# aipixel/GPS-Gaussian

Measured on NVIDIA H100. Metric: novel_views_per_sec_1024sq_500kgauss, higher is better.
Workload: dtype f32

## Files before the change

### gps-gaussian_b200/_lib.py

```python
import ctypes as C
import os
import threading

import torch

_HERE = os.path.dirname(os.path.abspath(__file__))
LIB_PATH = os.path.join(_HERE, "lib", "libgpsg_sm90.so")


class GpsgError(RuntimeError):
    pass


class RasterSettings(C.Structure):
    _fields_ = [("image_height", C.c_int32), ("image_width", C.c_int32), ("tanfovx", C.c_float),
                ("tanfovy", C.c_float), ("bg", C.c_float * 3), ("scale_modifier", C.c_float),
                ("viewmatrix", C.c_float * 16), ("projmatrix", C.c_float * 16), ("sh_degree", C.c_int32),
                ("campos", C.c_float * 3), ("prefiltered", C.c_int32), ("debug", C.c_int32)]


class GeomView(C.Structure):
    _fields_ = [("depths", C.c_void_p), ("means2D", C.c_void_p), ("conic_opacity", C.c_void_p),
                ("tiles_touched", C.c_void_p), ("point_offsets", C.c_void_p)]


class BinningView(C.Structure):
    _fields_ = [("point_list_keys", C.c_void_p), ("point_list", C.c_void_p), ("slabA", C.c_void_p), ("block_lists", C.c_void_p)]


class ImageView(C.Structure):
    _fields_ = [("final_T", C.c_void_p), ("n_contrib", C.c_void_p), ("ranges", C.c_void_p), ("block_counts", C.c_void_p)]


ALLOC_FN = C.CFUNCTYPE(C.c_void_p, C.c_void_p, C.c_size_t)

if not os.path.exists(LIB_PATH):
    raise ImportError(
        f"{LIB_PATH} not found: the CUDA extension is not built. Run `python gps-gaussian_b200/build.py` "
        "(nvcc, sm_90a). There is deliberately no CPU / PyTorch fallback.")

lib = C.CDLL(LIB_PATH)

_vp, _i, _i64, _sz = C.c_void_p, C.c_int, C.c_int64, C.c_size_t
lib.gpsg_last_error.restype = C.c_char_p
lib.gpsg_last_error.argtypes = []
lib.gpsg_version.restype = _i
_pp = C.POINTER(C.c_void_p)
_rs = C.POINTER(RasterSettings)
lib.gpsg_rasterize_forward.restype = _i
lib.gpsg_rasterize_forward.argtypes = [_rs, _i, _vp, _i, _i] + [_vp] * 11 + [
    ALLOC_FN, _vp, ALLOC_FN, _vp, ALLOC_FN, _vp, C.POINTER(C.c_int32), _i]
lib.gpsg_rasterize_forward_maps_begin.restype = _i
lib.gpsg_rasterize_forward_maps_begin.argtypes = [_rs, _i, _vp, _i] + [_pp] * 6 + [
    _vp, ALLOC_FN, _vp, ALLOC_FN, _vp, _vp, _i]
lib.gpsg_rasterize_forward_maps_finish.restype = _i
lib.gpsg_rasterize_forward_maps_finish.argtypes = [_rs, _i, _vp, _i] + [_pp] * 6 + [_vp] * 6 + [
    ALLOC_FN, _vp, _vp, C.POINTER(C.c_int32)]
lib.gpsg_rasterize_forward_planned.restype = _i
lib.gpsg_rasterize_forward_planned.argtypes = [_rs, _i, _vp, _i] + [_vp] * 12 + [_i64, _vp, _vp, _i]
lib.gpsg_rasterize_forward_maps_planned.restype = _i
lib.gpsg_rasterize_forward_maps_planned.argtypes = [_rs, _i, _vp, _i] + [_pp] * 6 + [_vp] * 6 + [_i64, _vp, _vp, _i]
lib.gpsg_rasterize_backward_workspace_bytes.restype = _sz
lib.gpsg_rasterize_backward_workspace_bytes.argtypes = [_i, _i64, _i, _i]
lib.gpsg_rasterize_backward.restype = _i
lib.gpsg_rasterize_backward.argtypes = [_rs, _i, _vp, _i, _i, C.c_int32] + [_vp] * 23 + [_i]
lib.gpsg_rasterize_backward_maps_workspace_bytes.restype = _sz
lib.gpsg_rasterize_backward_maps_workspace_bytes.argtypes = [_i, _i64, _i, _i]
lib.gpsg_rasterize_backward_maps.restype = _i
lib.gpsg_rasterize_backward_maps.argtypes = [_rs, _i, _vp, _i, C.c_int32] + [_pp] * 6 + [_vp] * 7 + [_pp] * 5 + [_vp, _i]
lib.gpsg_mark_visible.restype = _i
lib.gpsg_mark_visible.argtypes = [_i, _vp, _i, _vp, C.POINTER(C.c_float), _vp]
lib.gpsg_geom_view.restype = _i
lib.gpsg_geom_view.argtypes = [_vp, _i, C.POINTER(GeomView)]
lib.gpsg_binning_view.restype = _i
lib.gpsg_binning_view.argtypes = [_vp, _i64, C.POINTER(BinningView)]
lib.gpsg_image_view.restype = _i
lib.gpsg_image_view.argtypes = [_vp, _i, _i, C.POINTER(ImageView)]
lib.gpsg_corr_sampler_forward.restype = _i
lib.gpsg_corr_sampler_forward.argtypes = [_i, _vp, _i, _i, _i, _i, _i, _vp, _i64, _i64, _i64, _vp, _i64, _i, _vp]
lib.gpsg_corr_sampler_backward.restype = _i
lib.gpsg_corr_sampler_backward.argtypes = [_i, _vp, _i, _i, _i, _i, _i, _vp, _i64, _vp, _i, _vp]

lib.gpsg_raster_geom_bytes.restype = _sz
lib.gpsg_raster_geom_bytes.argtypes = [_i]
lib.gpsg_raster_binning_bytes.restype = _sz
lib.gpsg_raster_binning_bytes.argtypes = [_i64]
lib.gpsg_raster_image_bytes.restype = _sz
lib.gpsg_raster_image_bytes.argtypes = [_i, _i]
lib.gpsg_corr_build_pyramid.restype = _i
lib.gpsg_corr_build_pyramid.argtypes = [_i, _vp, _i, _i, _i, _i, _i, _i, _vp, _vp, C.POINTER(C.c_void_p), _i]
lib.gpsg_corr_build_backward.restype = _i
lib.gpsg_corr_build_backward.argtypes = [_i, _vp, _i, _i, _i, _i, _i, _i, _vp, _vp, _vp, _vp, _vp]
lib.gpsg_corr_lookup_pyramid_forward.restype = _i
lib.gpsg_corr_lookup_pyramid_forward.argtypes = [_i, _vp, _i, _i, _i, _i, C.POINTER(C.c_void_p), C.POINTER(C.c_int32), _i,
                                                 _vp, _i64, _i, _vp]
lib.gpsg_corr_lookup_pyramid_backward.restype = _i
lib.gpsg_corr_lookup_pyramid_backward.argtypes = [_i, _vp, _i, _i, _i, _i, C.POINTER(C.c_void_p), C.POINTER(C.c_int32), _i,
                                                  _vp, _i64, _i, _vp]
lib.gpsg_unproject_forward.restype = _i
lib.gpsg_unproject_forward.argtypes = [_i, _vp, _i, _i, _vp, _vp, _i64, _vp, _vp, _i, _vp, _vp, _vp, _vp, _vp]
lib.gpsg_unproject_backward.restype = _i
lib.gpsg_unproject_backward.argtypes = [_i, _vp, _i, _i, _vp, _vp, _i64, _vp, _vp, _i, _vp, _vp, _vp, _vp, _vp]
lib.gpsg_l1_ssim_workspace_bytes.restype = _sz
lib.gpsg_l1_ssim_workspace_bytes.argtypes = [_i, _i, _i]
lib.gpsg_l1_ssim_forward.restype = _i
lib.gpsg_l1_ssim_forward.argtypes = [_i, _vp, _i, _i, _i, _vp, _vp, C.c_float, C.c_float, _vp, _vp, _vp]
lib.gpsg_l1_ssim_backward.restype = _i
lib.gpsg_l1_ssim_backward.argtypes = [_i, _vp, _i, _i, _i, _vp, _vp, _vp, C.c_float, C.c_float, _vp, _vp]
lib.gpsg_point_splat_workspace_bytes.restype = _sz
lib.gpsg_point_splat_workspace_bytes.argtypes = [_i, _i]
lib.gpsg_point_splat.restype = _i
lib.gpsg_point_splat.argtypes = [_i, _vp, _i, _i, _i, _i64, _vp, _vp, _vp, _vp, _vp]


class RectifyCamera(C.Structure):
    _fields_ = [("K", C.c_double * 9), ("R", C.c_double * 9), ("P", C.c_double * 9)]


class RectifyPlanes(C.Structure):
    _fields_ = [(n, C.c_void_p) for n in ("img", "mask", "depth", "img_out", "mask_out", "depth_out", "img_tensor",
                                          "mask_tensor")]


MESH_MAX_CAMERAS = 8
MESH_MAX_LIGHTS = 16


class Mesh(C.Structure):
    _fields_ = [("verts", C.c_void_p), ("face_verts", C.c_void_p), ("uvs", C.c_void_p), ("face_uvs", C.c_void_p),
                ("tex", C.c_void_p), ("num_verts", C.c_int32), ("num_faces", C.c_int32), ("num_uvs", C.c_int32),
                ("tex_w", C.c_int32), ("tex_h", C.c_int32)]


class MeshCamera(C.Structure):
    _fields_ = [("width", C.c_int32), ("height", C.c_int32), ("fx", C.c_float), ("fy", C.c_float), ("cx", C.c_float),
                ("cy", C.c_float), ("pos", C.c_float * 3), ("inv_rot", C.c_float * 9), ("img", C.c_void_p),
                ("zbuf", C.c_void_p), ("mask", C.c_void_p)]


class MeshScene(C.Structure):
    _fields_ = [("cameras", MeshCamera * MESH_MAX_CAMERAS), ("light_dir", (C.c_float * 3) * MESH_MAX_LIGHTS),
                ("light_color", (C.c_float * 3) * MESH_MAX_LIGHTS), ("num_cameras", C.c_int32),
                ("num_lights", C.c_int32)]


lib.gpsg_mesh_render_workspace_bytes.restype = _sz
lib.gpsg_mesh_render_workspace_bytes.argtypes = [_i, _i64]
lib.gpsg_mesh_render.restype = _i
lib.gpsg_mesh_render.argtypes = [_i, _vp, Mesh, MeshScene, _vp, _sz]
lib.gpsg_rectify_remap.restype = _i
lib.gpsg_rectify_remap.argtypes = [_i, _vp, C.POINTER(RectifyCamera), _i, _i, _i, _i, _i, _i, C.POINTER(RectifyPlanes)]
lib.gpsg_rectify_flow.restype = _i
lib.gpsg_rectify_flow.argtypes = [_i, _vp, _i, _i, _i, C.c_double, C.c_double, C.c_double, _pp, _pp, _pp, _pp]
class SeqLossArgs(C.Structure):
    _fields_ = [("pred", C.c_void_p * 32), ("grad", C.c_void_p * 32), ("weight", C.c_float * 32), ("gt", C.c_void_p),
                ("valid", C.c_void_p), ("numel", C.c_int64), ("n_pred", C.c_int), ("gt_dtype", C.c_int)]


SEQ_LOSS_MAX_PRED = 32
GS_HEAD_PARAMS = ("out_w", "out_b", "rot_w1", "rot_b1", "rot_w2", "rot_b2", "scale_w1", "scale_b1", "scale_w2",
                  "scale_b2", "opacity_w1", "opacity_b1", "opacity_w2", "opacity_b2")
lib.gpsg_convex_upsample_forward.restype = _i
lib.gpsg_convex_upsample_forward.argtypes = [_i, _vp, _i, _i, _i, _i, _i, _i, _vp, _vp, _vp]
lib.gpsg_convex_upsample_backward_workspace_bytes.restype = _sz
lib.gpsg_convex_upsample_backward_workspace_bytes.argtypes = [_i, _i, _i, _i]
lib.gpsg_convex_upsample_backward.restype = _i
lib.gpsg_convex_upsample_backward.argtypes = [_i, _vp, _i, _i, _i, _i, _i, _i, _vp, _vp, _vp, _vp, _vp, _vp]
lib.gpsg_sequence_loss_workspace_bytes.restype = _sz
lib.gpsg_sequence_loss_workspace_bytes.argtypes = []
lib.gpsg_sequence_loss_forward.restype = _i
lib.gpsg_sequence_loss_forward.argtypes = [_i, _vp, SeqLossArgs, _vp, _vp]
lib.gpsg_sequence_loss_backward.restype = _i
lib.gpsg_sequence_loss_backward.argtypes = [_i, _vp, SeqLossArgs, _vp, _vp]


class GsHeadWeights(C.Structure):
    _fields_ = [(n, C.c_void_p) for n in GS_HEAD_PARAMS]


lib.gpsg_gs_head_workspace_bytes.restype = _sz
lib.gpsg_gs_head_workspace_bytes.argtypes = [_i, _i, _i]
lib.gpsg_gs_head_forward.restype = _i
lib.gpsg_gs_head_forward.argtypes = [_i, _vp, _i, _i, _i] + [_vp] * 6 + [GsHeadWeights, _vp]


class GsHeadGrads(C.Structure):
    _fields_ = [(n, C.c_void_p) for n in GS_HEAD_PARAMS]


lib.gpsg_gs_head_backward_workspace_bytes.restype = _sz
lib.gpsg_gs_head_backward_workspace_bytes.argtypes = [_i, _i, _i]
lib.gpsg_gs_head_backward.restype = _i
lib.gpsg_gs_head_backward.argtypes = [_i, _vp, _i, _i, _i] + [_vp] * 9 + [GsHeadWeights, GsHeadGrads, _vp]
ENCODER_STEM_PARAMS = ("in_conv_w", "in_conv_b", "in_norm_w", "in_norm_b") + tuple(
    f"b{k}_{n}" for k in (1, 2) for n in ("conv1_w", "conv1_b", "norm1_w", "norm1_b", "conv2_w", "conv2_b", "norm2_w",
                                          "norm2_b"))
ENCODER_STEM_TF32, ENCODER_STEM_FP16 = 0, 1


class EncoderStemWeights(C.Structure):
    _fields_ = [(n, C.c_void_p) for n in ENCODER_STEM_PARAMS]


lib.gpsg_encoder_stem_workspace_bytes.restype = _sz
lib.gpsg_encoder_stem_workspace_bytes.argtypes = [_i, _i, _i, _i, _i]
lib.gpsg_encoder_stem_forward.restype = _i
lib.gpsg_encoder_stem_forward.argtypes = [_i, _vp, _i, _i, _i, _i, _i, _vp, EncoderStemWeights, _vp, _vp]
lib.gpsg_profile_enable.restype = _i
lib.gpsg_profile_enable.argtypes = [_i]
lib.gpsg_profile_read.restype = _i
lib.gpsg_profile_read.argtypes = [C.POINTER(C.c_float), C.POINTER(C.c_int32), C.POINTER(C.c_int32), _i]
lib.gpsg_profile_stage_name.restype = C.c_char_p
lib.gpsg_profile_stage_name.argtypes = [_i]

EXPORTED = ["gpsg_last_error", "gpsg_version", "gpsg_rasterize_forward", "gpsg_rasterize_forward_maps_begin",
            "gpsg_rasterize_forward_maps_finish", "gpsg_raster_geom_bytes", "gpsg_raster_binning_bytes",
            "gpsg_raster_image_bytes", "gpsg_rasterize_forward_planned", "gpsg_rasterize_forward_maps_planned",
            "gpsg_rasterize_backward_workspace_bytes", "gpsg_rasterize_backward",
            "gpsg_rasterize_backward_maps_workspace_bytes", "gpsg_rasterize_backward_maps", "gpsg_mark_visible",
            "gpsg_geom_view", "gpsg_binning_view", "gpsg_image_view", "gpsg_corr_sampler_forward",
            "gpsg_corr_sampler_backward", "gpsg_corr_build_pyramid", "gpsg_corr_build_backward",
            "gpsg_corr_lookup_pyramid_forward", "gpsg_corr_lookup_pyramid_backward", "gpsg_unproject_forward",
            "gpsg_unproject_backward", "gpsg_l1_ssim_workspace_bytes", "gpsg_l1_ssim_forward", "gpsg_l1_ssim_backward",
            "gpsg_set_corr_build", "gpsg_profile_enable", "gpsg_profile_read", "gpsg_profile_stage_name",
            "gpsg_point_splat_workspace_bytes", "gpsg_point_splat", "gpsg_rectify_remap", "gpsg_rectify_flow",
            "gpsg_convex_upsample_forward", "gpsg_convex_upsample_backward_workspace_bytes",
            "gpsg_convex_upsample_backward", "gpsg_sequence_loss_workspace_bytes", "gpsg_sequence_loss_forward",
            "gpsg_sequence_loss_backward", "gpsg_mesh_render_workspace_bytes", "gpsg_mesh_render", "gpsg_jpeg_parse",
            "gpsg_jpeg_decode_workspace_bytes", "gpsg_jpeg_decode", "gpsg_jpeg_encode_max_bytes",
            "gpsg_jpeg_encode_workspace_bytes", "gpsg_jpeg_encode", "gpsg_gs_head_workspace_bytes",
            "gpsg_gs_head_forward", "gpsg_gs_head_backward_workspace_bytes", "gpsg_gs_head_backward",
            "gpsg_encoder_stem_workspace_bytes", "gpsg_encoder_stem_forward"]

BWD_DETERMINISTIC = 1
FWD_ANTIALIAS = 1


def forward_flags(antialiasing=False):
    return FWD_ANTIALIAS if antialiasing else 0


def check(rc, what):
    if rc != 0:
        msg = lib.gpsg_last_error()
        raise GpsgError(f"{what} failed (code {rc}): {msg.decode() if msg else ''}")


_tls = threading.local()


def _alloc_trampoline(user, nbytes):
    try:
        t = torch.empty(int(nbytes), dtype=torch.uint8, device=_tls.device)
        _tls.bufs[int(user or 0)] = t
        return t.data_ptr()
    except Exception:
        return None


ALLOC_CB = ALLOC_FN(_alloc_trampoline)


def begin_alloc(device):
    _tls.device = device
    _tls.bufs = {}


def end_alloc():
    bufs = _tls.bufs
    _tls.bufs = {}
    return bufs


def device_stream(device):
    device = torch.device(device)
    idx = device.index if device.index is not None else torch.cuda.current_device()
    return idx, C.c_void_p(torch.cuda.current_stream(idx).cuda_stream)


def _ptr(t):
    return C.c_void_p(t.data_ptr()) if (t is not None and t.numel() > 0) else None


def rasterize_forward(settings, out_color, radii, means3D, opacities, colors_precomp=None, shs=None, scales=None,
                      rotations=None, cov3D_precomp=None, out_depth=None, out_alpha=None, antialiasing=False):
    if (out_depth is None) != (out_alpha is None):
        raise ValueError("out_depth and out_alpha must be given together")
    dev = means3D.device
    idx, stream = device_stream(dev)
    n = C.c_int32(0)
    fn = lib.gpsg_rasterize_forward
    begin_alloc(dev)
    try:
        with torch.cuda.device(dev):
            rc = fn(
                C.byref(settings), idx, stream, int(means3D.shape[0]), int(shs.shape[1]) if shs is not None else 0,
                _ptr(means3D), _ptr(colors_precomp), _ptr(shs), _ptr(opacities), _ptr(scales), _ptr(rotations),
                _ptr(cov3D_precomp), _ptr(out_color), _ptr(out_depth), _ptr(out_alpha), _ptr(radii), ALLOC_CB, C.c_void_p(1),
                ALLOC_CB, C.c_void_p(2), ALLOC_CB, C.c_void_p(3), C.byref(n), forward_flags(antialiasing))
    finally:
        bufs = end_alloc()
    check(rc, fn.__name__)
    return int(n.value), (bufs.get(1), bufs.get(2), bufs.get(3))


def backward_flags(deterministic=None):
    if deterministic is None:
        deterministic = torch.are_deterministic_algorithms_enabled()
    return BWD_DETERMINISTIC if deterministic else 0

# ... 55 lines not shown
```

### gps-gaussian_b200/build.py

```python
import os
import subprocess
import sys
from concurrent.futures import ThreadPoolExecutor

HERE = os.path.dirname(os.path.abspath(__file__))
CSRC = os.path.join(HERE, "csrc")
OBJ = os.path.join(HERE, "build")
LIBDIR = os.path.join(HERE, "lib")
LIB = os.path.join(LIBDIR, "libgpsg_sm90.so")

ARCH = ["-gencode", "arch=compute_90a,code=sm_90a"]
COMMON = ["-O3", "-std=c++17", "-lineinfo", "-Xcompiler", "-fPIC", "-Xcompiler", "-fvisibility=hidden",
          "--expt-relaxed-constexpr", "-Xptxas", "-v"]
SOURCES = {
    "gpsg_capi.cu": [],
    "raster_preprocess.cu": ["-fmad=false"],
    "raster_binning.cu": [],
    "raster_render.cu": [],
    "raster_backward.cu": [],
    "corr.cu": [],
    "corr_tc.cu": [],
    "sh.cu": [],
    "unproject.cu": [],
    "loss.cu": [],
    "point_splat.cu": [],
    "rectify.cu": ["-fmad=false"],
    "flow_head.cu": [],
    "gs_head.cu": [],
    "encoder_stem.cu": [],
    "mesh_render.cu": ["-fmad=false"],
    "jpeg_decode.cu": [],
    "jpeg_encode.cu": [],
}


def _nvcc():
    for cand in (os.environ.get("NVCC"), "/usr/local/cuda/bin/nvcc", "nvcc"):
        if cand and (os.path.isabs(cand) and os.path.exists(cand) or not os.path.isabs(cand)):
            return cand
    return "nvcc"


def _deps(src):
    hdrs = [os.path.join(CSRC, f) for f in os.listdir(CSRC) if f.endswith((".cuh", ".h"))]
    hdrs.append(os.path.join(os.path.dirname(HERE), "include", "gpsg.h"))
    return [src, os.path.abspath(__file__)] + hdrs


def _stale(dst, deps):
    if not os.path.exists(dst):
        return True
    t = os.path.getmtime(dst)
    return any(os.path.getmtime(d) > t for d in deps)


def _compile(name, extra, force, verbose):
    src = os.path.join(CSRC, name)
    obj = os.path.join(OBJ, name.replace(".cu", ".o"))
    if not force and not _stale(obj, _deps(src)):
        return obj, ""
    cmd = [_nvcc()] + ARCH + COMMON + extra + ["-c", src, "-o", obj]
    p = subprocess.run(cmd, capture_output=True, text=True)
    log = " ".join(cmd) + "\n" + p.stdout + p.stderr
    if p.returncode != 0:
        raise RuntimeError(log)
    with open(obj + ".log", "w") as f:
        f.write(log)
    if verbose:
        print(log)
    return obj, log


def build(force=False, verbose=False):
    os.makedirs(OBJ, exist_ok=True)
    os.makedirs(LIBDIR, exist_ok=True)
    with ThreadPoolExecutor(max_workers=len(SOURCES)) as ex:
        res = list(ex.map(lambda kv: _compile(kv[0], kv[1], force, verbose), SOURCES.items()))
    objs = [r[0] for r in res]
    if force or _stale(LIB, objs):
        cmd = [_nvcc()] + ARCH + ["-shared", "-o", LIB] + objs + ["-Xcompiler", "-fvisibility=hidden", "-cudart",
                                                                  "static"]
        p = subprocess.run(cmd, capture_output=True, text=True)
        if p.returncode != 0:
            raise RuntimeError(" ".join(cmd) + "\n" + p.stdout + p.stderr)
    return LIB


if __name__ == "__main__":
    print(build(force="--force" in sys.argv, verbose="--verbose" in sys.argv))
```

### gps-gaussian_b200/csrc/raster_binning.cu

```cuda
#include <cub/cub.cuh>
#include "gpsg_internal.cuh"
#include "tile_scan.cuh"

namespace gpsg {

size_t scan_temp_bytes(int P) {
    size_t bytes = 0;
    cub::DeviceScan::InclusiveSum(nullptr, bytes, (uint32_t*)nullptr, (uint32_t*)nullptr, P > 0 ? P : 1);
    return bytes;
}

size_t sort_temp_bytes(size_t N, int end_bit) {
    size_t bytes = 0;
    cub::DeviceRadixSort::SortPairs(nullptr, bytes, (uint64_t*)nullptr, (uint64_t*)nullptr, (uint32_t*)nullptr,
                                    (uint32_t*)nullptr, (int64_t)(N > 0 ? N : 1), 0, end_bit);
    return bytes;
}

int run_scan(GeomState g, int P, cudaStream_t stream) {
    if (P <= 0) return GPSG_OK;
    size_t bytes = g.scan_temp_bytes;
    GPSG_CUDA(cub::DeviceScan::InclusiveSum(g.scan_temp, bytes, g.tiles_touched, g.point_offsets, P, stream));
    return GPSG_OK;
}

__global__ void __launch_bounds__(256) duplicate_kernel(const __grid_constant__ Camera cam, int P,
                                                        const int32_t* __restrict__ radii, GeomState g,
                                                        BinningState b) {
    const int i = blockIdx.x * blockDim.x + threadIdx.x;
    if (i >= P) return;
    const int radius = radii[i];
    if (radius <= 0) return;
    uint32_t off = (i == 0) ? 0u : g.point_offsets[i - 1];
    int rx0, ry0, rx1, ry1;
    tile_rect(cam.grid_x, cam.grid_y, g.means2D[i], radius, rx0, ry0, rx1, ry1);
    const uint64_t dbits = (uint64_t)__float_as_uint(g.depths[i]);
    for (int y = ry0; y < ry1; ++y)
        for (int x = rx0; x < rx1; ++x) {
            const uint64_t key = ((uint64_t)(uint32_t)(y * cam.grid_x + x) << 32) | dbits;
            b.keys_unsorted[off] = key;
            b.vals_unsorted[off] = (uint32_t)i;
            ++off;
        }
}

int launch_duplicate(const Camera& cam, int P, const int32_t* radii, GeomState g, BinningState b, cudaStream_t stream) {
    if (P <= 0) return GPSG_OK;
    duplicate_kernel<<<(P + 255) / 256, 256, 0, stream>>>(cam, P, radii, g, b);
    GPSG_LAUNCH_CHECK();
    return GPSG_OK;
}

int run_sort(BinningState b, size_t N, int end_bit, cudaStream_t stream) {
    if (N == 0) return GPSG_OK;
    size_t bytes = b.sort_temp_bytes;
    GPSG_CUDA(cub::DeviceRadixSort::SortPairs(b.sort_temp, bytes, b.keys_unsorted, b.keys, b.vals_unsorted, b.vals,
                                              (int64_t)N, 0, end_bit, stream));
    return GPSG_OK;
}



__global__ void __launch_bounds__(256) tile_scan_kernel(int tiles, ImageState im, uint32_t capacity) {
    tile_scan_block(tiles, im, capacity);
}

int launch_tile_scan(const Camera& cam, ImageState im, uint32_t capacity, cudaStream_t stream) {
    tile_scan_kernel<<<1, 256, 0, stream>>>(cam.grid_x * cam.grid_y, im, capacity);
    GPSG_LAUNCH_CHECK();
    return GPSG_OK;
}

__global__ void __launch_bounds__(256) bucket_scatter_kernel(const __grid_constant__ Camera cam, int P,
                                                             const int32_t* __restrict__ radii, GeomState g,
                                                             BinningState b, ImageState im) {
    __shared__ uint32_t sh_cnt[kBoxBins];
    __shared__ uint32_t sh_base[kBoxBins];
    __shared__ int s_bb[4];
    if (im.totals[2]) return;
    if (threadIdx.x == 0) { s_bb[0] = 0x7fffffff; s_bb[1] = 0x7fffffff; s_bb[2] = 0; s_bb[3] = 0; }
    for (int t = threadIdx.x; t < kBoxBins; t += blockDim.x) sh_cnt[t] = 0u;
    __syncthreads();
    const int i = blockIdx.x * blockDim.x + threadIdx.x;
    int rx0 = 0, ry0 = 0, rx1 = 0, ry1 = 0;
    uint2 entry = make_uint2(0u, 0u);
    if (i < P) {
        const int radius = radii[i];
        if (radius > 0) {
            tile_rect(cam.grid_x, cam.grid_y, g.means2D[i], radius, rx0, ry0, rx1, ry1);
            entry = make_uint2((uint32_t)i, __float_as_uint(g.depths[i]));
        }
    }
    TileBox box;
    if (!cta_tile_box(rx0, ry0, rx1, ry1, s_bb, box)) {
        for (int y = ry0; y < ry1; ++y)
            for (int x = rx0; x < rx1; ++x) {
                const int t = y * cam.grid_x + x;
                b.bucket[im.ranges[t].x + atomicAdd(&im.tile_cursor[t], 1u)] = entry;
            }
        return;
    }
    for (int y = ry0; y < ry1; ++y)
        for (int x = rx0; x < rx1; ++x) atomicAdd(&sh_cnt[(y - box.y0) * box.w + (x - box.x0)], 1u);
    __syncthreads();
    for (int t = threadIdx.x; t < box.w * box.h; t += blockDim.x) {
        const uint32_t c = sh_cnt[t];
        if (c) {
            const int tile = (box.y0 + t / box.w) * cam.grid_x + box.x0 + t % box.w;
            sh_base[t] = im.ranges[tile].x + atomicAdd(&im.tile_cursor[tile], c);
            sh_cnt[t] = 0u;
        }
    }
    __syncthreads();
    for (int y = ry0; y < ry1; ++y)
        for (int x = rx0; x < rx1; ++x) {
            const int t = (y - box.y0) * box.w + (x - box.x0);
            b.bucket[sh_base[t] + atomicAdd(&sh_cnt[t], 1u)] = entry;
        }
}

int launch_bucket_scatter(const Camera& cam, int P, const int32_t* radii, GeomState g, BinningState b, ImageState im,
                          cudaStream_t stream) {
    if (P <= 0) return GPSG_OK;
    bucket_scatter_kernel<<<(P + 255) / 256, 256, 0, stream>>>(cam, P, radii, g, b, im);
    GPSG_LAUNCH_CHECK();
    return GPSG_OK;
}

__device__ __forceinline__ void slab_entry(uint32_t id, const GaussianSrc& src, const GeomState& g, float4& A,
                                           float4& B, float4& C) {
    const float2 xy = g.means2D[id];
    const float4 co = g.conic_opacity[id];
    float r, gg, bb;
    src_color(src, id, r, gg, bb);
    float ex = 3.0e38f, ey = 3.0e38f;
    const float detc = co.x * co.z - co.y * co.y;
    if (!(co.w * 255.0f >= 1.0f)) {
        ex = ey = -3.0e38f;
    } else if (detc > 0.0f && co.x > 0.0f && co.z > 0.0f) {
        const float tau2 = 2.0f * __logf(co.w * 255.0f) * 1.0005f + 1e-4f;
        ex = sqrtf(tau2 * co.z / detc) * 1.0005f + 0.01f;
        ey = sqrtf(tau2 * co.x / detc) * 1.0005f + 0.01f;
        if (!(ex == ex) || !(ey == ey)) { ex = 3.0e38f; ey = 3.0e38f; }
    }
    A = make_float4(xy.x, xy.y, ex, ey);
    const float kL = 1.4426950408889634f;
    B = make_float4(-0.5f * kL * co.x, -kL * co.y, -0.5f * kL * co.z, co.w);
    C = make_float4(r, gg, bb, __uint_as_float(id));
}

constexpr int kSortThreads = 512;
constexpr int kSortCTAsPerSM = 3;


__device__ __forceinline__ uint32_t block_hit_mask(const float4& a, int tile_x, int tile_y) {
    bool hx[2], hy[4];
#pragma unroll
    for (int c = 0; c < 2; ++c) {
        const float wx0 = (float)(tile_x * GPSG_TILE_X + 8 * c), wx1 = (float)(tile_x * GPSG_TILE_X + 8 * c + 7);
        hx[c] = (a.x >= wx0 - a.z) && (a.x <= wx1 + a.z);
    }
#pragma unroll
    for (int w = 0; w < 4; ++w) {
        const float wy0 = (float)(tile_y * GPSG_TILE_Y + 4 * w), wy1 = (float)(tile_y * GPSG_TILE_Y + 4 * w + 3);
        hy[w] = (a.y >= wy0 - a.w) && (a.y <= wy1 + a.w);
    }
    uint32_t hits = 0u;
#pragma unroll
    for (int k = 0; k < 8; ++k) hits |= (uint32_t)(hx[fwd_block_col(k)] && hy[fwd_block_row(k)]) << k;
    return hits;
}

__device__ __forceinline__ void append_block_list(const uint8_t* hits, uint32_t r0, uint32_t m, int k,
                                                  uint32_t* __restrict__ list, uint32_t& base) {
    const int lane = threadIdx.x & 31;
    const unsigned lt = (1u << lane) - 1u;
#pragma unroll 4
    for (uint32_t c = 0; c < m; c += 32) {
        const uint32_t i = c + lane;
        const bool hit = i < m && ((hits[i] >> k) & 1u);
        const unsigned mask = __ballot_sync(0xffffffffu, hit);
        if (hit) list[base + __popc(mask & lt)] = r0 + i;
        base += __popc(mask);
    }
}

constexpr int kBigItems = (int)kMaxTileSort / kSortThreads;
template <int ITEMS>
struct TileSort {
    using BRS = cub::BlockRadixSort<uint32_t, kSortThreads, ITEMS, uint32_t, 4, false>;
    union Smem {
        typename BRS::TempStorage sort;
        unsigned long long keys[kSortThreads * ITEMS];
    };

    static constexpr int kMaxRun = 16;
    __device__ static void run(Smem& sm, uint32_t* flags, uint8_t* hits, const uint2* __restrict__ src, int n, int id_bits,
                               uint32_t tile, int grid_x, size_t out0, const GaussianSrc& src_in, const GeomState& g,
                               const BinningState& b, uint32_t* __restrict__ blk_count) {
        uint32_t keys[ITEMS], ids[ITEMS];
        uint32_t dmin = ~0u, dmax = 0u;
#pragma unroll
        for (int k = 0; k < ITEMS; ++k) {
            const int i = k * kSortThreads + (int)threadIdx.x;
            const uint2 e = i < n ? src[i] : make_uint2(0u, 0u);
            ids[k] = e.x;
            keys[k] = e.y;
            if (i < n) { dmin = min(dmin, e.y); dmax = max(dmax, e.y); }
        }
        dmin = __reduce_min_sync(0xffffffffu, dmin);
        dmax = __reduce_max_sync(0xffffffffu, dmax);
        if (threadIdx.x == 0) { flags[0] = ~0u; flags[1] = 0u; flags[2] = 0u; }
        __syncthreads();
        if ((threadIdx.x & 31) == 0) { atomicMin(&flags[0], dmin); atomicMax(&flags[1], dmax); }
        __syncthreads();
        const uint32_t dlo = flags[0];
        const int w = 32 - __clz(flags[1] - dlo);
        const uint32_t pad = 1u << w;
#pragma unroll
        for (int k = 0; k < ITEMS; ++k) keys[k] = (k * kSortThreads + (int)threadIdx.x) < n ? keys[k] - dlo : pad;
        BRS(sm.sort).SortBlockedToStriped(keys, ids, 0, w + 1);
        __syncthreads();
#pragma unroll
        for (int k = 0; k < ITEMS; ++k)
            sm.keys[k * kSortThreads + (int)threadIdx.x] = ((unsigned long long)(keys[k] + dlo) << 32) | ids[k];
        __syncthreads();
        bool redo = false;
#pragma unroll 1
        for (int k = 0; k < ITEMS; ++k) {
            const int r = k * kSortThreads + (int)threadIdx.x;
            if (r + 1 < n) {
                const uint32_t d = (uint32_t)(sm.keys[r] >> 32);
                const bool start = (r == 0 || (uint32_t)(sm.keys[r - 1] >> 32) != d) && (uint32_t)(sm.keys[r + 1] >> 32) == d;
                if (start) {
                    int e = r + 1;
                    while (e + 1 < n && (uint32_t)(sm.keys[e + 1] >> 32) == d) ++e;
                    if (e - r + 1 > kMaxRun) redo = true;
                    else
                        for (int a = r + 1; a <= e; ++a) {
                            const unsigned long long v = sm.keys[a];
                            int c = a - 1;
                            while (c >= r && sm.keys[c] > v) { sm.keys[c + 1] = sm.keys[c]; --c; }
                            sm.keys[c + 1] = v;
                        }
                }
            }
        }
        if (redo) flags[2] = 1u;
        __syncthreads();
        if (flags[2]) {
#pragma unroll
            for (int k = 0; k < ITEMS; ++k) {
                const int r = k * kSortThreads + (int)threadIdx.x;
                const unsigned long long v = sm.keys[r];
                ids[k] = (uint32_t)v;
                keys[k] = r < n ? (uint32_t)(v >> 32) - dlo : pad;
            }
            __syncthreads();
            BRS(sm.sort).SortBlockedToStriped(ids, keys, 0, id_bits);
            __syncthreads();
#pragma unroll
            for (int k = 0; k < ITEMS; ++k)
                sm.keys[k * kSortThreads + (int)threadIdx.x] = ((unsigned long long)keys[k] << 32) | ids[k];
            __syncthreads();
#pragma unroll
            for (int k = 0; k < ITEMS; ++k) {
                const unsigned long long v = sm.keys[(int)threadIdx.x * ITEMS + k];
                ids[k] = (uint32_t)v;
                keys[k] = (uint32_t)(v >> 32);
            }
            __syncthreads();
            BRS(sm.sort).SortBlockedToStriped(keys, ids, 0, w + 1);
            __syncthreads();
#pragma unroll
            for (int k = 0; k < ITEMS; ++k)
                sm.keys[k * kSortThreads + (int)threadIdx.x] = ((unsigned long long)(keys[k] + dlo) << 32) | ids[k];
            __syncthreads();
        }
        const unsigned long long tile_hi = (unsigned long long)tile << 32;
        const int tile_y = (int)tile / grid_x, tile_x = (int)tile - tile_y * grid_x;
#pragma unroll 1
        for (int k = 0; k < ITEMS; ++k) {
            const int r = k * kSortThreads + (int)threadIdx.x;
            if (r < n) {
                const unsigned long long v = sm.keys[r];
                const uint32_t id = (uint32_t)v;
                const size_t o = out0 + r;
                if (b.keys) {
                    b.keys[o] = tile_hi | (v >> 32);
                    b.vals[o] = id;
                }
                float4 A, B, C;
                slab_entry(id, src_in, g, A, B, C);
                b.slabA[o] = A;
                b.slabB[o] = B;
                b.slabC[o] = C;
                hits[r] = (uint8_t)block_hit_mask(A, tile_x, tile_y);
            }
        }
        __syncthreads();
        const int warp = (int)threadIdx.x >> 5, blk = warp & 7;
        const uint32_t split = ((uint32_t)n / 2u) & ~127u;
        uint32_t* __restrict__ list = b.blk_list + 8 * out0 + (size_t)blk * n;
        uint32_t cnt = 0u;
        if (warp < 8) {
            append_block_list(hits, 0u, split, blk, list, cnt);
        } else {
            const uint32_t* __restrict__ words = reinterpret_cast<const uint32_t*>(hits);
#pragma unroll 1
            for (uint32_t i = threadIdx.x & 31; i < split / 4u; i += 32) cnt += __popc(words[i] & (0x01010101u << blk));
            cnt = __reduce_add_sync(0xffffffffu, cnt);
            append_block_list(hits + split, split, (uint32_t)n - split, blk, list, cnt);
            if ((threadIdx.x & 31) == 0) blk_count[8 * (size_t)tile + blk] = cnt;
        }
    }
};

template <bool BIG>
__global__ void __launch_bounds__(kSortThreads, BIG ? 1 : kSortCTAsPerSM) tile_sort_gather_kernel(const GaussianSrc colors, GeomState g,
                                                                            BinningState b, ImageState im, int id_bits,
                                                                            int grid_x, uint32_t tiles) {
    __shared__ uint32_t flags[4];
    if (im.totals[2]) return;
    if constexpr (BIG) {
        __shared__ typename TileSort<kBigItems>::Smem t16;
        __shared__ __align__(16) uint8_t hits[kSortThreads * kBigItems];
        const uint32_t nbig = im.totals[3];
        for (uint32_t k = blockIdx.x; k < nbig; k += gridDim.x) {
            const uint32_t tile = im.big_tiles[k];
            const uint2 range = im.ranges[tile];
            const int n = (int)(range.y - range.x);
            TileSort<kBigItems>::run(t16, flags, hits, b.bucket + range.x, n, id_bits, tile, grid_x, range.x, colors, g, b,
                                     im.blk_count);
            __syncthreads();
        }
    } else {
        __shared__ union {
            typename TileSort<1>::Smem t1;
            typename TileSort<2>::Smem t2;
            typename TileSort<3>::Smem t3;
            typename TileSort<4>::Smem t4;
        } temp;
        __shared__ __align__(16) uint8_t hits[kSortThreads * 4];
#pragma unroll 1
        for (;;) {
            if (threadIdx.x == 0) flags[3] = atomicAdd(&im.totals[kSortTicketWord], 1u);
            __syncthreads();
            const uint32_t i = flags[3];
            if (i >= tiles) break;
            const uint32_t tile = im.tile_order[i];
            const uint2 range = im.ranges[tile];
            const int n = (int)(range.y - range.x);
            if (n == 0) break;
            const uint2* __restrict__ src = b.bucket + range.x;
            if (n <= 512) TileSort<1>::run(temp.t1, flags, hits, src, n, id_bits, tile, grid_x, range.x, colors, g, b, im.blk_count);
            else if (n <= 1024) TileSort<2>::run(temp.t2, flags, hits, src, n, id_bits, tile, grid_x, range.x, colors, g, b, im.blk_count);
            else if (n <= 1536) TileSort<3>::run(temp.t3, flags, hits, src, n, id_bits, tile, grid_x, range.x, colors, g, b, im.blk_count);
            else if (n <= (int)kBigTile) TileSort<4>::run(temp.t4, flags, hits, src, n, id_bits, tile, grid_x, range.x, colors, g, b, im.blk_count);
            __syncthreads();
        }
    }
}

constexpr int kBigTileCTAs = 132;

int launch_tile_sort_gather(const Camera& cam, int P, uint32_t max_count, const GaussianSrc& colors, GeomState g,
                            BinningState b, ImageState im, cudaStream_t stream) {
    int id_bits = 1;
    while (id_bits < 32 && (1ll << id_bits) < (long long)P) ++id_bits;
    const int tiles = cam.grid_x * cam.grid_y;
    const int ctas = resident_grid((const void*)tile_sort_gather_kernel<false>, kSortThreads);
    GPSG_REQUIRE(ctas > 0, "tile sort: could not query the occupancy of tile_sort_gather_kernel on the current device");
    tile_sort_gather_kernel<false><<<min(tiles, ctas), kSortThreads, 0, stream>>>(colors, g, b, im, id_bits, cam.grid_x,
                                                                                   (uint32_t)tiles);
    GPSG_LAUNCH_CHECK();
    if (max_count > kBigTile) {
        tile_sort_gather_kernel<true><<<min(tiles, kBigTileCTAs), kSortThreads, 0, stream>>>(colors, g, b, im, id_bits,
                                                                                             cam.grid_x, (uint32_t)tiles);
        GPSG_LAUNCH_CHECK();
    }
    return GPSG_OK;
}

__global__ void __launch_bounds__(256) gather_ranges_kernel(size_t N, const GaussianSrc colors, GeomState g,
                                                            BinningState b, ImageState im) {
    const size_t i = (size_t)blockIdx.x * blockDim.x + threadIdx.x;
    if (i >= N) return;
    const uint64_t key = b.keys[i];
    const uint32_t tile = (uint32_t)(key >> 32);
    if (i == 0) {
        im.ranges[tile].x = 0;
    } else {
        const uint32_t prev = (uint32_t)(b.keys[i - 1] >> 32);
        if (prev != tile) {
            im.ranges[prev].y = (uint32_t)i;
            im.ranges[tile].x = (uint32_t)i;
        }
    }
    if (i == N - 1) im.ranges[tile].y = (uint32_t)N;
    const uint32_t id = b.vals[i];
    float4 A, B, C;
    slab_entry(id, colors, g, A, B, C);
    b.slabA[i] = A;
    b.slabB[i] = B;
    b.slabC[i] = C;
}

constexpr uint32_t kListChunk = 8 * kSortThreads;
__global__ void __launch_bounds__(kSortThreads) block_lists_kernel(int grid_x, BinningState b, ImageState im) {
    __shared__ uint8_t hits[kListChunk];
    const uint32_t tile = blockIdx.x;
    const uint2 range = im.ranges[tile];
    const uint32_t n = range.y - range.x;
    if (n == 0) return;
    const int tile_y = (int)tile / grid_x, tile_x = (int)tile - tile_y * grid_x;
    const float4* __restrict__ tileA = b.slabA + range.x;
    const int warp = (int)threadIdx.x >> 5;
    uint32_t* __restrict__ list = b.blk_list + 8 * (size_t)range.x + (size_t)min(warp, 7) * n;
    uint32_t cnt = 0u;
#pragma unroll 1
    for (uint32_t r0 = 0; r0 < n; r0 += kListChunk) {
        const uint32_t m = min(kListChunk, n - r0);
        for (uint32_t i = threadIdx.x; i < m; i += kSortThreads) hits[i] = (uint8_t)block_hit_mask(tileA[r0 + i], tile_x, tile_y);
        __syncthreads();
        if (warp < 8) append_block_list(hits, r0, m, warp, list, cnt);
        __syncthreads();
    }
    if (warp < 8 && (threadIdx.x & 31) == 0) im.blk_count[8 * (size_t)tile + warp] = cnt;
}

int launch_gather_ranges(const Camera& cam, size_t N, const GaussianSrc& colors, GeomState g, BinningState b, ImageState im,
                         cudaStream_t stream) {
    const int tiles = cam.grid_x * cam.grid_y;
    GPSG_CUDA(cudaMemsetAsync(im.ranges, 0, sizeof(uint2) * (size_t)tiles, stream));
    if (N == 0) return GPSG_OK;
    gather_ranges_kernel<<<(unsigned)((N + 255) / 256), 256, 0, stream>>>(N, colors, g, b, im);
    GPSG_LAUNCH_CHECK();
    block_lists_kernel<<<tiles, kSortThreads, 0, stream>>>(cam.grid_x, b, im);
    GPSG_LAUNCH_CHECK();
    return GPSG_OK;
}

}
```

### gps-gaussian_b200/csrc/sm90_ptx.cuh

```cuda
#pragma once
#include <stdint.h>

namespace gpsg {
namespace sm90 {

__device__ __forceinline__ uint32_t smem_addr(const void* p) { return (uint32_t)__cvta_generic_to_shared(p); }

__device__ __forceinline__ float tf32(float x) {
    uint32_t r;
    asm("cvt.rna.tf32.f32 %0, %1;" : "=r"(r) : "f"(x));
    return __uint_as_float(r);
}

__device__ __forceinline__ float ex2_approx(float x) {
    float y;
    asm("ex2.approx.ftz.f32 %0, %1;" : "=f"(y) : "f"(x));
    return y;
}

__device__ __forceinline__ float rcp_approx(float x) {
    float y;
    asm("rcp.approx.ftz.f32 %0, %1;" : "=f"(y) : "f"(x));
    return y;
}

__device__ __forceinline__ uint32_t opaque(uint32_t x) {
    uint32_t y;
    asm volatile("mov.u32 %0, %1;" : "=r"(y) : "r"(x));
    return y;
}

__device__ __forceinline__ uint64_t gmma_desc(uint32_t addr, uint32_t lbo_bytes, uint32_t sbo_bytes) {
    uint64_t d = 0;
    d |= (uint64_t)((addr & 0x3FFFFu) >> 4);
    d |= (uint64_t)((lbo_bytes >> 4) & 0x3FFFu) << 16;
    d |= (uint64_t)((sbo_bytes >> 4) & 0x3FFFu) << 32;
    return d;
}

__device__ __forceinline__ void wgmma_m64n32k8(float (&d)[16], uint64_t a_desc, uint64_t b_desc) {
    asm volatile(
        "{\n\t.reg .pred p;\n\tsetp.ne.b32 p, %18, 0;\n\t"
        "wgmma.mma_async.sync.aligned.m64n32k8.f32.tf32.tf32 "
        "{%0, %1, %2, %3, %4, %5, %6, %7, %8, %9, %10, %11, %12, %13, %14, %15}, %16, %17, p, 1, 1;\n\t}"
        : "+f"(d[0]), "+f"(d[1]), "+f"(d[2]), "+f"(d[3]), "+f"(d[4]), "+f"(d[5]), "+f"(d[6]), "+f"(d[7]), "+f"(d[8]), "+f"(d[9]), "+f"(d[10]), "+f"(d[11]), "+f"(d[12]), "+f"(d[13]), "+f"(d[14]), "+f"(d[15])
        : "l"(a_desc), "l"(b_desc), "n"(1)
        : "memory");
}

__device__ __forceinline__ void wgmma_m64n56k8(float (&d)[28], uint64_t a_desc, uint64_t b_desc) {
    asm volatile(
        "{\n\t.reg .pred p;\n\tsetp.ne.b32 p, %30, 0;\n\t"
        "wgmma.mma_async.sync.aligned.m64n56k8.f32.tf32.tf32 "
        "{%0, %1, %2, %3, %4, %5, %6, %7, %8, %9, %10, %11, %12, %13, %14, %15, %16, %17, %18, %19, %20, %21, %22, %23, %24, %25, %26, %27}, %28, %29, p, 1, 1;\n\t}"
        : "+f"(d[0]), "+f"(d[1]), "+f"(d[2]), "+f"(d[3]), "+f"(d[4]), "+f"(d[5]), "+f"(d[6]), "+f"(d[7]), "+f"(d[8]), "+f"(d[9]), "+f"(d[10]), "+f"(d[11]), "+f"(d[12]), "+f"(d[13]), "+f"(d[14]), "+f"(d[15]), "+f"(d[16]), "+f"(d[17]), "+f"(d[18]), "+f"(d[19]), "+f"(d[20]), "+f"(d[21]), "+f"(d[22]), "+f"(d[23]), "+f"(d[24]), "+f"(d[25]), "+f"(d[26]), "+f"(d[27])
        : "l"(a_desc), "l"(b_desc), "n"(1)
        : "memory");
}

__device__ __forceinline__ void wgmma_m64n96k8(float (&d)[48], uint64_t a_desc, uint64_t b_desc) {
    asm volatile(
        "{\n\t.reg .pred p;\n\tsetp.ne.b32 p, %50, 0;\n\t"
        "wgmma.mma_async.sync.aligned.m64n96k8.f32.tf32.tf32 "
        "{%0, %1, %2, %3, %4, %5, %6, %7, %8, %9, %10, %11, %12, %13, %14, %15, %16, %17, %18, %19, %20, %21, %22, %23, %24, %25, %26, %27, %28, %29, %30, %31, %32, %33, %34, %35, %36, %37, %38, %39, %40, %41, %42, %43, %44, %45, %46, %47}, %48, %49, p, 1, 1;\n\t}"
        : "+f"(d[0]), "+f"(d[1]), "+f"(d[2]), "+f"(d[3]), "+f"(d[4]), "+f"(d[5]), "+f"(d[6]), "+f"(d[7]), "+f"(d[8]), "+f"(d[9]), "+f"(d[10]), "+f"(d[11]), "+f"(d[12]), "+f"(d[13]), "+f"(d[14]), "+f"(d[15]), "+f"(d[16]), "+f"(d[17]), "+f"(d[18]), "+f"(d[19]), "+f"(d[20]), "+f"(d[21]), "+f"(d[22]), "+f"(d[23]), "+f"(d[24]), "+f"(d[25]), "+f"(d[26]), "+f"(d[27]), "+f"(d[28]), "+f"(d[29]), "+f"(d[30]), "+f"(d[31]), "+f"(d[32]), "+f"(d[33]), "+f"(d[34]), "+f"(d[35]), "+f"(d[36]), "+f"(d[37]), "+f"(d[38]), "+f"(d[39]), "+f"(d[40]), "+f"(d[41]), "+f"(d[42]), "+f"(d[43]), "+f"(d[44]), "+f"(d[45]), "+f"(d[46]), "+f"(d[47])
        : "l"(a_desc), "l"(b_desc), "n"(1)
        : "memory");
}

template <int TA, int TB>
__device__ __forceinline__ void wgmma_m64n16k16_f16(float (&d)[8], uint64_t a_desc, uint64_t b_desc, int accumulate) {
    asm volatile(
        "{\n\t.reg .pred p;\n\t"
        "setp.ne.b32 p, %10, 0;\n\t"
        "wgmma.mma_async.sync.aligned.m64n16k16.f32.f16.f16 {%0, %1, %2, %3, %4, %5, %6, %7}, %8, %9, p, 1, 1, %11, %12;\n\t}"
        : "+f"(d[0]), "+f"(d[1]), "+f"(d[2]), "+f"(d[3]), "+f"(d[4]), "+f"(d[5]), "+f"(d[6]), "+f"(d[7])
        : "l"(a_desc), "l"(b_desc), "r"(accumulate), "n"(TA), "n"(TB)
        : "memory");
}

__device__ __forceinline__ void wgmma_m64n32k16_f16(float (&d)[16], uint64_t a_desc, uint64_t b_desc) {
    asm volatile(
        "{\n\t.reg .pred p;\n\tsetp.ne.b32 p, %18, 0;\n\t"
        "wgmma.mma_async.sync.aligned.m64n32k16.f32.f16.f16 "
        "{%0, %1, %2, %3, %4, %5, %6, %7, %8, %9, %10, %11, %12, %13, %14, %15}, %16, %17, p, 1, 1, 0, 0;\n\t}"
        : "+f"(d[0]), "+f"(d[1]), "+f"(d[2]), "+f"(d[3]), "+f"(d[4]), "+f"(d[5]), "+f"(d[6]), "+f"(d[7]), "+f"(d[8]), "+f"(d[9]), "+f"(d[10]), "+f"(d[11]), "+f"(d[12]), "+f"(d[13]), "+f"(d[14]), "+f"(d[15])
        : "l"(a_desc), "l"(b_desc), "n"(1)
        : "memory");
}

template <int N>
__device__ __forceinline__ void fence_acc(float (&acc)[N]) {
#pragma unroll
    for (int i = 0; i < N; ++i) asm volatile("" : "+f"(acc[i])::"memory");
}
template <int NC>
__device__ __forceinline__ void fence_acc(float (&acc)[NC][8]) {
#pragma unroll
    for (int c = 0; c < NC; ++c) fence_acc(acc[c]);
}

__device__ __forceinline__ void wgmma_fence() { asm volatile("wgmma.fence.sync.aligned;" ::: "memory"); }
__device__ __forceinline__ void wgmma_commit() { asm volatile("wgmma.commit_group.sync.aligned;" ::: "memory"); }
__device__ __forceinline__ void wgmma_wait() { asm volatile("wgmma.wait_group.sync.aligned 0;" ::: "memory"); }
__device__ __forceinline__ void fence_async() { asm volatile("fence.proxy.async.shared::cta;" ::: "memory"); }

__device__ __forceinline__ void mma_m16n8k8(float (&d)[4], const float (&a)[4], float b0, float b1) {
    asm volatile("mma.sync.aligned.m16n8k8.row.col.f32.tf32.tf32.f32 {%0, %1, %2, %3}, {%4, %5, %6, %7}, {%8, %9}, "
                 "{%0, %1, %2, %3};"
                 : "+f"(d[0]), "+f"(d[1]), "+f"(d[2]), "+f"(d[3])
                 : "r"(__float_as_uint(a[0])), "r"(__float_as_uint(a[1])), "r"(__float_as_uint(a[2])),
                   "r"(__float_as_uint(a[3])), "r"(__float_as_uint(b0)), "r"(__float_as_uint(b1)));
}

__device__ __forceinline__ void cp_async16(void* smem, const void* gmem) {
    asm volatile("cp.async.cg.shared.global [%0], [%1], 16;" ::"r"(smem_addr(smem)), "l"(gmem) : "memory");
}
__device__ __forceinline__ void cp_async16_zfill(void* smem, const void* gmem, uint32_t src_bytes) {
    asm volatile("cp.async.cg.shared.global [%0], [%1], 16, %2;" ::"r"(smem_addr(smem)), "l"(gmem), "r"(src_bytes)
                 : "memory");
}
__device__ __forceinline__ void cp_async4(void* smem, const void* gmem) {
    asm volatile("cp.async.ca.shared.global [%0], [%1], 4;" ::"r"(smem_addr(smem)), "l"(gmem) : "memory");
}
__device__ __forceinline__ void cp_async_commit() { asm volatile("cp.async.commit_group;" ::: "memory"); }
__device__ __forceinline__ void cp_async_wait1() { asm volatile("cp.async.wait_group 1;" ::: "memory"); }
__device__ __forceinline__ void cp_async_wait_all() { asm volatile("cp.async.wait_all;" ::: "memory"); }

}
}
```

Measured before the change: 5246.

## Add counting-sort fast path for small tile sorts, with optional phase timers

For tiles with at most 4 items per thread, keys are bucketed by depth into 2048 shared-memory counters, prefix-scanned, scattered, and each bucket is finished with an insertion sort. If any bucket holds more than 32 entries, the kernel reloads the inputs and falls back to the existing CUB block radix sort. The aim is to replace multi-pass radix sorting with a single histogram-and-scatter pass. In exchange the shared-memory footprint grows, which may lower occupancy, and skewed depth distributions pay for both paths. Compile-time phase timers via globaltimer and a build option for extra defines are also added.

After: 5644 (median of 6 runs). 1.08x the previous value.

```diff
diff --git a/gps-gaussian_b200/_lib.py b/gps-gaussian_b200/_lib.py
--- a/gps-gaussian_b200/_lib.py
+++ b/gps-gaussian_b200/_lib.py
@@ -5,7 +5,7 @@
 import torch
 
 _HERE = os.path.dirname(os.path.abspath(__file__))
-LIB_PATH = os.path.join(_HERE, "lib", "libgpsg_sm90.so")
+LIB_PATH = os.environ.get("GPSG_LIB_PATH") or os.path.join(_HERE, "lib", "libgpsg_sm90.so")
 
 
 class GpsgError(RuntimeError):
diff --git a/gps-gaussian_b200/build.py b/gps-gaussian_b200/build.py
--- a/gps-gaussian_b200/build.py
+++ b/gps-gaussian_b200/build.py
@@ -54,9 +54,9 @@
     return any(os.path.getmtime(d) > t for d in deps)
 
 
-def _compile(name, extra, force, verbose):
+def _compile(name, extra, objdir, force, verbose):
     src = os.path.join(CSRC, name)
-    obj = os.path.join(OBJ, name.replace(".cu", ".o"))
+    obj = os.path.join(objdir, name.replace(".cu", ".o"))
     if not force and not _stale(obj, _deps(src)):
         return obj, ""
     cmd = [_nvcc()] + ARCH + COMMON + extra + ["-c", src, "-o", obj]
@@ -71,19 +71,22 @@
     return obj, log
 
 
-def build(force=False, verbose=False):
-    os.makedirs(OBJ, exist_ok=True)
-    os.makedirs(LIBDIR, exist_ok=True)
+def build(force=False, verbose=False, defines=(), out=None):
+    objdir = os.path.join(OBJ, "_".join(defines)) if defines else OBJ
+    lib = out or LIB
+    flags = ["-D" + d for d in defines]
+    os.makedirs(objdir, exist_ok=True)
+    os.makedirs(os.path.dirname(lib), exist_ok=True)
     with ThreadPoolExecutor(max_workers=len(SOURCES)) as ex:
-        res = list(ex.map(lambda kv: _compile(kv[0], kv[1], force, verbose), SOURCES.items()))
+        res = list(ex.map(lambda kv: _compile(kv[0], kv[1] + flags, objdir, force, verbose), SOURCES.items()))
     objs = [r[0] for r in res]
-    if force or _stale(LIB, objs):
-        cmd = [_nvcc()] + ARCH + ["-shared", "-o", LIB] + objs + ["-Xcompiler", "-fvisibility=hidden", "-cudart",
+    if force or _stale(lib, objs):
+        cmd = [_nvcc()] + ARCH + ["-shared", "-o", lib] + objs + ["-Xcompiler", "-fvisibility=hidden", "-cudart",
                                                                   "static"]
         p = subprocess.run(cmd, capture_output=True, text=True)
         if p.returncode != 0:
             raise RuntimeError(" ".join(cmd) + "\n" + p.stdout + p.stderr)
-    return LIB
+    return lib
 
 
 if __name__ == "__main__":
diff --git a/gps-gaussian_b200/csrc/raster_binning.cu b/gps-gaussian_b200/csrc/raster_binning.cu
--- a/gps-gaussian_b200/csrc/raster_binning.cu
+++ b/gps-gaussian_b200/csrc/raster_binning.cu
@@ -1,6 +1,8 @@
 #include <cub/cub.cuh>
+#include <type_traits>
 #include "gpsg_internal.cuh"
 #include "tile_scan.cuh"
+#include "sm90_ptx.cuh"
 
 namespace gpsg {
 
@@ -152,6 +154,30 @@
 constexpr int kSortThreads = 512;
 constexpr int kSortCTAsPerSM = 3;
 
+#ifdef GPSG_SORT_PHASES
+__device__ unsigned long long g_sort_phase_ns[8];
+__shared__ unsigned long long s_sort_clock;
+#define SORT_PHASE(k)                                                                                      \
+    do {                                                                                                   \
+        if (threadIdx.x == 0) {                                                                            \
+            const unsigned long long now_ = sm90::globaltimer();                                           \
+            if ((k) >= 0) atomicAdd(&g_sort_phase_ns[(k) < 0 ? 0 : (k)], now_ - s_sort_clock);             \
+            if ((k) == 0) atomicAdd(&g_sort_phase_ns[6], 1ull);                                            \
+            s_sort_clock = now_;                                                                           \
+        }                                                                                                  \
+    } while (0)
+
+extern "C" GPSG_API int gpsg_sort_phases_read(unsigned long long* out) {
+    GPSG_CUDA(cudaDeviceSynchronize());
+    GPSG_CUDA(cudaMemcpyFromSymbol(out, g_sort_phase_ns, sizeof(g_sort_phase_ns)));
+    const unsigned long long zero[8] = {};
+    GPSG_CUDA(cudaMemcpyToSymbol(g_sort_phase_ns, zero, sizeof(zero)));
+    return GPSG_OK;
+}
+#else
+#define SORT_PHASE(k) do {} while (0)
+#endif
+
 
 __device__ __forceinline__ uint32_t block_hit_mask(const float4& a, int tile_x, int tile_y) {
     bool hx[2], hy[4];
@@ -189,12 +215,68 @@
 template <int ITEMS>
 struct TileSort {
     using BRS = cub::BlockRadixSort<uint32_t, kSortThreads, ITEMS, uint32_t, 4, false>;
-    union Smem {
-        typename BRS::TempStorage sort;
-        unsigned long long keys[kSortThreads * ITEMS];
+    static constexpr bool kCounting = ITEMS <= 4;
+    static constexpr int kBucketBits = 11, kBuckets = 1 << kBucketBits;
+    static_assert(kBuckets == 4 * kSortThreads, "the counter scan gives each thread 4 buckets");
+    struct CountingSmem {
+        __align__(16) uint32_t cnt[kBuckets];
+        uint32_t warp_sum[kSortThreads / 32];
     };
-
+    struct Smem {
+        union {
+            typename BRS::TempStorage sort;
+            unsigned long long keys[kSortThreads * ITEMS];
+        };
+        std::conditional_t<kCounting, CountingSmem, cub::NullType> c;
+    };
+
+    static constexpr int kMaxBucket = 32;
     static constexpr int kMaxRun = 16;
+
+    __device__ static bool count_sort(Smem& sm, uint32_t* flags, const uint32_t (&keys)[ITEMS],
+                                      const uint32_t (&ids)[ITEMS], int n, uint32_t dlo, int w) {
+        CountingSmem& c = sm.c;
+        const int shift = max(0, w - kBucketBits);
+        const int lane = (int)threadIdx.x & 31, warp = (int)threadIdx.x >> 5;
+#pragma unroll
+        for (int k = 0; k < ITEMS; ++k)
+            if (k * kSortThreads + (int)threadIdx.x < n) atomicAdd(&c.cnt[(keys[k] - dlo) >> shift], 1u);
+        __syncthreads();
+        const uint4 q = reinterpret_cast<const uint4*>(c.cnt)[threadIdx.x];
+        const uint32_t sum = q.x + q.y + q.z + q.w;
+        uint32_t incl = sum;
+#pragma unroll
+        for (int d = 1; d < 32; d <<= 1) {
+            const uint32_t v = __shfl_up_sync(0xffffffffu, incl, d);
+            if (lane >= d) incl += v;
+        }
+        if (lane == 31) c.warp_sum[warp] = incl;
+        if (max(max(q.x, q.y), max(q.z, q.w)) > (uint32_t)kMaxBucket) flags[3] = 1u;
+        __syncthreads();
+        const uint32_t base = __reduce_add_sync(0xffffffffu, lane < warp ? c.warp_sum[lane] : 0u) + incl - sum;
+        reinterpret_cast<uint4*>(c.cnt)[threadIdx.x] = make_uint4(base, base + q.x, base + q.x + q.y, base + q.x + q.y + q.z);
+        const bool ok = flags[3] == 0u;
+        __syncthreads();
+        if (!ok) return false;
+#pragma unroll
+        for (int k = 0; k < ITEMS; ++k)
+            if (k * kSortThreads + (int)threadIdx.x < n)
+                sm.keys[atomicAdd(&c.cnt[(keys[k] - dlo) >> shift], 1u)] = ((unsigned long long)keys[k] << 32) | ids[k];
+        __syncthreads();
+#pragma unroll 1
+        for (int j = 4 * (int)threadIdx.x; j < 4 * (int)threadIdx.x + 4; ++j) {
+            const int r = j ? (int)c.cnt[j - 1] : 0, e = (int)c.cnt[j];
+            for (int a = r + 1; a < e; ++a) {
+                const unsigned long long v = sm.keys[a];
+                int d = a - 1;
+                while (d >= r && sm.keys[d] > v) { sm.keys[d + 1] = sm.keys[d]; --d; }
+                sm.keys[d + 1] = v;
+            }
+        }
+        __syncthreads();
+        return true;
+    }
+
     __device__ static void run(Smem& sm, uint32_t* flags, uint8_t* hits, const uint2* __restrict__ src, int n, int id_bits,
                                uint32_t tile, int grid_x, size_t out0, const GaussianSrc& src_in, const GeomState& g,
                                const BinningState& b, uint32_t* __restrict__ blk_count) {
@@ -210,12 +292,35 @@
         }
         dmin = __reduce_min_sync(0xffffffffu, dmin);
         dmax = __reduce_max_sync(0xffffffffu, dmax);
-        if (threadIdx.x == 0) { flags[0] = ~0u; flags[1] = 0u; flags[2] = 0u; }
+        if (threadIdx.x == 0) { flags[0] = ~0u; flags[1] = 0u; flags[2] = 0u; flags[3] = 0u; }
+        if constexpr (kCounting) reinterpret_cast<uint4*>(sm.c.cnt)[threadIdx.x] = make_uint4(0u, 0u, 0u, 0u);
         __syncthreads();
         if ((threadIdx.x & 31) == 0) { atomicMin(&flags[0], dmin); atomicMax(&flags[1], dmax); }
         __syncthreads();
+        SORT_PHASE(1);
         const uint32_t dlo = flags[0];
         const int w = 32 - __clz(flags[1] - dlo);
+        bool sorted = false;
+        if constexpr (kCounting) sorted = count_sort(sm, flags, keys, ids, n, dlo, w);
+        SORT_PHASE(2);
+        if (!sorted) {
+            if constexpr (kCounting) {
+#pragma unroll
+                for (int k = 0; k < ITEMS; ++k) {
+                    const int i = k * kSortThreads + (int)threadIdx.x;
+                    const uint2 e = i < n ? src[i] : make_uint2(0u, 0u);
+                    ids[k] = e.x;
+                    keys[k] = e.y;
+                }
+            }
+            radix_sort(sm, flags, keys, ids, n, id_bits, dlo, w);
+        }
+        SORT_PHASE(3);
+        gather_and_lists(sm, hits, n, tile, grid_x, out0, src_in, g, b, blk_count);
+    }
+
+    __device__ static void radix_sort(Smem& sm, uint32_t* flags, uint32_t (&keys)[ITEMS], uint32_t (&ids)[ITEMS], int n,
+                                      int id_bits, uint32_t dlo, int w) {
         const uint32_t pad = 1u << w;
 #pragma unroll
         for (int k = 0; k < ITEMS; ++k) keys[k] = (k * kSortThreads + (int)threadIdx.x) < n ? keys[k] - dlo : pad;
@@ -277,6 +382,11 @@
                 sm.keys[k * kSortThreads + (int)threadIdx.x] = ((unsigned long long)(keys[k] + dlo) << 32) | ids[k];
             __syncthreads();
         }
+    }
+
+    __device__ static void gather_and_lists(Smem& sm, uint8_t* hits, int n, uint32_t tile, int grid_x, size_t out0,
+                                            const GaussianSrc& src_in, const GeomState& g, const BinningState& b,
+                                            uint32_t* __restrict__ blk_count) {
         const unsigned long long tile_hi = (unsigned long long)tile << 32;
         const int tile_y = (int)tile / grid_x, tile_x = (int)tile - tile_y * grid_x;
 #pragma unroll 1
@@ -299,6 +409,7 @@
             }
         }
         __syncthreads();
+        SORT_PHASE(4);
         const int warp = (int)threadIdx.x >> 5, blk = warp & 7;
         const uint32_t split = ((uint32_t)n / 2u) & ~127u;
         uint32_t* __restrict__ list = b.blk_list + 8 * out0 + (size_t)blk * n;
@@ -320,19 +431,22 @@
 __global__ void __launch_bounds__(kSortThreads, BIG ? 1 : kSortCTAsPerSM) tile_sort_gather_kernel(const GaussianSrc colors, GeomState g,
                                                                             BinningState b, ImageState im, int id_bits,
                                                                             int grid_x, uint32_t tiles) {
-    __shared__ uint32_t flags[4];
+    __shared__ uint32_t flags[5];
     if (im.totals[2]) return;
     if constexpr (BIG) {
         __shared__ typename TileSort<kBigItems>::Smem t16;
         __shared__ __align__(16) uint8_t hits[kSortThreads * kBigItems];
         const uint32_t nbig = im.totals[3];
+        SORT_PHASE(-1);
         for (uint32_t k = blockIdx.x; k < nbig; k += gridDim.x) {
             const uint32_t tile = im.big_tiles[k];
             const uint2 range = im.ranges[tile];
             const int n = (int)(range.y - range.x);
+            SORT_PHASE(0);
             TileSort<kBigItems>::run(t16, flags, hits, b.bucket + range.x, n, id_bits, tile, grid_x, range.x, colors, g, b,
                                      im.blk_count);
             __syncthreads();
+            SORT_PHASE(5);
         }
     } else {
         __shared__ union {
@@ -342,22 +456,25 @@
             typename TileSort<4>::Smem t4;
         } temp;
         __shared__ __align__(16) uint8_t hits[kSortThreads * 4];
+        SORT_PHASE(-1);
 #pragma unroll 1
         for (;;) {
-            if (threadIdx.x == 0) flags[3] = atomicAdd(&im.totals[kSortTicketWord], 1u);
-            __syncthreads();
-            const uint32_t i = flags[3];
+            if (threadIdx.x == 0) flags[4] = atomicAdd(&im.totals[kSortTicketWord], 1u);
+            __syncthreads();
+            const uint32_t i = flags[4];
             if (i >= tiles) break;
             const uint32_t tile = im.tile_order[i];
             const uint2 range = im.ranges[tile];
             const int n = (int)(range.y - range.x);
             if (n == 0) break;
             const uint2* __restrict__ src = b.bucket + range.x;
+            SORT_PHASE(0);
             if (n <= 512) TileSort<1>::run(temp.t1, flags, hits, src, n, id_bits, tile, grid_x, range.x, colors, g, b, im.blk_count);
             else if (n <= 1024) TileSort<2>::run(temp.t2, flags, hits, src, n, id_bits, tile, grid_x, range.x, colors, g, b, im.blk_count);
             else if (n <= 1536) TileSort<3>::run(temp.t3, flags, hits, src, n, id_bits, tile, grid_x, range.x, colors, g, b, im.blk_count);
             else if (n <= (int)kBigTile) TileSort<4>::run(temp.t4, flags, hits, src, n, id_bits, tile, grid_x, range.x, colors, g, b, im.blk_count);
             __syncthreads();
+            SORT_PHASE(5);
         }
     }
 }
diff --git a/gps-gaussian_b200/csrc/sm90_ptx.cuh b/gps-gaussian_b200/csrc/sm90_ptx.cuh
--- a/gps-gaussian_b200/csrc/sm90_ptx.cuh
+++ b/gps-gaussian_b200/csrc/sm90_ptx.cuh
@@ -28,6 +28,12 @@
     uint32_t y;
     asm volatile("mov.u32 %0, %1;" : "=r"(y) : "r"(x));
     return y;
+}
+
+__device__ __forceinline__ unsigned long long globaltimer() {
+    unsigned long long t;
+    asm volatile("mov.u64 %0, %%globaltimer;" : "=l"(t));
+    return t;
 }
 
 __device__ __forceinline__ uint64_t gmma_desc(uint32_t addr, uint32_t lbo_bytes, uint32_t sbo_bytes) {
```
